# databricks/spark-deep-learning

Hardware: AMD Instinct MI355X
Metric: images/sec (higher is better)
Workload: dtype bf16; 1 GPU; model=resnet50, global_batch=512, image=224, parallelism=dp1

## Files before the change

### sparkdl/models/resnet.py

```python

import torch
import torch.nn as nn

from sparkdl.ops import BatchNormAct2d, Conv1x1, batch_norm_relu_maxpool


class Bottleneck(nn.Module):
    expansion = 4

    def __init__(self, cin, width, stride=1):
        super().__init__()
        cout = width * self.expansion
        self.conv1 = Conv1x1(cin, width)
        self.bn1 = BatchNormAct2d(width, relu=True)
        self.conv2 = nn.Conv2d(width, width, 3, stride=stride, padding=1,
                               bias=False)
        self.bn2 = BatchNormAct2d(width, relu=True)
        self.conv3 = Conv1x1(width, cout)
        self.bn3 = BatchNormAct2d(cout, relu=True)
        if stride != 1 or cin != cout:
            self.down_conv = Conv1x1(cin, cout, stride=stride)
            self.down_bn = BatchNormAct2d(cout, relu=False)
        else:
            self.down_conv = None

    def forward(self, x):
        x, skip = x if isinstance(x, tuple) else (x, x)
        if self.down_conv is not None:
            idn = self.down_bn(self.down_conv(skip))
        else:
            idn = skip
        out = self.bn1(self.conv1(x))
        out = self.bn2(self.conv2(out))
        return self.bn3(self.conv3(out), residual=idn, fork=True)


class ResNet50(nn.Module):
    LAYERS = (3, 4, 6, 3)

    def __init__(self, num_classes=1000):
        super().__init__()
        self.stem_conv = nn.Conv2d(3, 64, 7, stride=2, padding=3,
                                   bias=False)
        self.stem_bn = BatchNormAct2d(64, relu=True)
        self.stem_pool = nn.MaxPool2d(3, stride=2, padding=1)
        cin = 64
        stages = []
        for i, blocks in enumerate(self.LAYERS):
            width = 64 * (2 ** i)
            stride = 1 if i == 0 else 2
            layer = []
            for b in range(blocks):
                layer.append(Bottleneck(cin, width, stride if b == 0 else 1))
                cin = width * Bottleneck.expansion
            stages.append(nn.Sequential(*layer))
        self.stages = nn.Sequential(*stages)
        self.pool = nn.AdaptiveAvgPool2d(1)
        self.fc = nn.Linear(2048, num_classes)

        for m in self.modules():
            if isinstance(m, nn.Conv2d):
                nn.init.kaiming_normal_(m.weight, mode="fan_out",
                                        nonlinearity="relu")
        for m in self.modules():
            if isinstance(m, Bottleneck):
                nn.init.zeros_(m.bn3.weight)

    def forward(self, x):
        bn = self.stem_bn
        x = batch_norm_relu_maxpool(
            self.stem_conv(x), bn.weight, bn.bias, bn.running_mean,
            bn.running_var, momentum=bn.momentum, eps=bn.eps,
            training=bn.training)
        x, _ = self.stages(x)
        x = self.pool(x).flatten(1)
        return self.fc(x)
```

### sparkdl/ops/__init__.py

```python

_EXT = None
_EXT_ERR = None


def ext():
    global _EXT, _EXT_ERR
    if _EXT is None and _EXT_ERR is None:
        try:
            from sparkdl import _C
            _EXT = _C
        except ImportError as e:
            _EXT_ERR = e
    if _EXT is None:
        raise RuntimeError(
            "sparkdl._C HIP extension is not built. Run "
            "`python setup.py build_ext --inplace` (gfx950). "
            "Original error: %s" % _EXT_ERR)
    return _EXT


def has_ext():
    try:
        ext()
        return True
    except RuntimeError:
        return False


from sparkdl.ops.functional import (
    layer_norm, bias_gelu, batch_norm_act, batch_norm_relu_maxpool,
    layer_norm_ref, bias_gelu_ref,
    flash_attention, flash_attention_packed, masked_attention_ref,
    seqlens_from_mask, dropout_add_layer_norm, dropout_keep_mask,
)
from sparkdl.ops.modules import (
    LayerNorm, Linear, LinearGelu, Conv1x1, BatchNormAct2d,
    DropoutAddLayerNorm, convert_bf16_training,
)
from sparkdl.ops.optim import FusedAdamW, FusedSGD
```

### sparkdl/ops/csrc/batchnorm.hip

```cpp

#include "common.hip.h"
#include "kernels.h"

namespace {

constexpr int kBlock = 256;
constexpr int kVec = 8;
constexpr int kUnroll = 2;
constexpr int kFoldFloats = kBlock * 2 * kVec;
constexpr int kFinCh = 4;

__device__ __forceinline__ float bn_affine(short x, float scale,
                                           float shift) {
  return bf2f(x) * scale + shift;
}
__device__ __forceinline__ float bn_xhat(short x, float mean, float rstd) {
  return (bf2f(x) - mean) * rstd;
}
__device__ __forceinline__ float bn_dx(float d, float xh, float k1,
                                       float k2, float k3) {
  return k1 * (d - k2 - xh * k3);
}


// ... 675 lines not shown
      const float k2 = j < 4 ? b0[j] : b1[j - 4];
      const float k3 = j < 4 ? g0[j] : g1[j - 4];
      odx[j] = f2bf(bn_dx(d[j], xh, k1, k2, k3));
    }
    *(short8*)(dx + base) = odx;
  }
}

int bn_grid(long long rows, int cols) {
  const int tpr = cols / kVec;
  const int rpb = kBlock / min(tpr, kBlock);
  long long blocks = (rows + rpb - 1) / rpb;
  return (int)min(blocks, 2048LL);
}

}

int bn_reduce_blocks(long long rows, int cols) {
  const int tpr = cols / kVec;
  const int rpb = kBlock / min(tpr, kBlock);
  const long long row_blocks = (rows + rpb - 1) / rpb;
  const long long g = max(256LL, min(512LL, rows / 64));
  return (int)max(1LL, min(row_blocks, g));
}

long long bn_scratch_floats(long long rows, int cols) {
  return (long long)bn_reduce_blocks(rows, cols) * 2 * cols + 3LL * cols;
}

void launch_bn_fwd(const short* x, const short* res, const float* gamma,
                   const float* beta, float* running_mean,
                   float* running_var, float* save_mean, float* save_rstd,
                   float* scratch, short* y, unsigned char* mask,
                   long long rows, int cols, float momentum, float eps,
                   bool training, bool relu, hipStream_t stream) {
  const int grid = bn_grid(rows, cols);
  const int G = bn_reduce_blocks(rows, cols);
  if (training)
    hipLaunchKernelGGL(bn_stats_k<kUnroll>, dim3(G), dim3(kBlock), 0,
                       stream, x, scratch, rows, cols);
  float* scale = scratch + (size_t)G * 2 * cols;
  float* shift = scale + cols;
  hipLaunchKernelGGL(bn_finalize_k, dim3(cols / kFinCh), dim3(kBlock), 0,
                     stream, scratch, G, gamma, beta, running_mean,
                     running_var, save_mean, save_rstd, scale, shift, rows,
                     cols, momentum, eps, (int)training);
  auto ap = relu ? (res ? bn_apply_k<true, true> : bn_apply_k<true, false>)
                 : (res ? bn_apply_k<false, true>
                        : bn_apply_k<false, false>);
  hipLaunchKernelGGL(ap, dim3(grid), dim3(kBlock), 0, stream, x, res,
                     scale, shift, y, mask, rows, cols);
}

void launch_bn_bwd(const short* x, const unsigned char* mask,
                   const short* dy, const float* gamma,
                   const float* save_mean, const float* save_rstd,
                   float* scratch, float* dgamma, float* dbeta, short* dx,
                   short* dres, long long rows, int cols, bool training,
                   bool relu, hipStream_t stream) {
  const int grid = bn_grid(rows, cols);
  const int G = bn_reduce_blocks(rows, cols);
  auto rk = relu ? bn_bwd_reduce_k<true, kUnroll>
                 : bn_bwd_reduce_k<false, kUnroll>;
  hipLaunchKernelGGL(rk, dim3(G), dim3(kBlock), 0, stream, x, mask, dy,
                     save_mean, save_rstd, scratch, rows, cols);
  float* c1 = scratch + (size_t)G * 2 * cols;
  float* c2 = c1 + cols;
  float* c3 = c2 + cols;
  hipLaunchKernelGGL(bn_bwd_finalize_k, dim3(cols / kFinCh), dim3(kBlock),
                     0, stream, scratch, G, gamma, save_rstd, dgamma, dbeta,
                     c1, c2, c3, rows, cols, (int)training);
  auto ak = relu ? (dres ? bn_bwd_apply_k<true, true>
                         : bn_bwd_apply_k<true, false>)
                 : (dres ? bn_bwd_apply_k<false, true>
                         : bn_bwd_apply_k<false, false>);
  hipLaunchKernelGGL(ak, dim3(grid), dim3(kBlock), 0, stream, x, mask, dy,
                     save_mean, save_rstd, c1, c2, c3, dx, dres, rows,
                     cols);
}

void launch_bn_bwd2(const short* x, const unsigned char* mask,
                    const short* dya, const short* dyb, const float* gamma,
                    const float* save_mean, const float* save_rstd,
                    float* scratch, float* dgamma, float* dbeta, short* dx,
                    short* s, long long rows, int cols, bool training,
                    bool relu, hipStream_t stream) {
  const int grid = bn_grid(rows, cols);
  const int G = bn_reduce_blocks(rows, cols);
  auto rk = relu ? bn_bwd2_reduce_k<true, kUnroll>
                 : bn_bwd2_reduce_k<false, kUnroll>;
  hipLaunchKernelGGL(rk, dim3(G), dim3(kBlock), 0, stream, x, mask, dya,
                     dyb, save_mean, save_rstd, s, scratch, rows, cols);
  float* c1 = scratch + (size_t)G * 2 * cols;
  float* c2 = c1 + cols;
  float* c3 = c2 + cols;
  hipLaunchKernelGGL(bn_bwd_finalize_k, dim3(cols / kFinCh), dim3(kBlock),
                     0, stream, scratch, G, gamma, save_rstd, dgamma, dbeta,
                     c1, c2, c3, rows, cols, (int)training);
  hipLaunchKernelGGL(bn_bwd2_apply_k, dim3(grid), dim3(kBlock), 0, stream,
                     x, s, save_mean, save_rstd, c1, c2, c3, dx, rows,
                     cols);
}

void launch_bn_pool_fwd(const short* x, const float* gamma,
                        const float* beta, float* running_mean,
                        float* running_var, float* save_mean,
// ... 45 lines not shown
```

### sparkdl/ops/csrc/bindings.cpp

```cpp

#include <torch/extension.h>
#include <ATen/hip/impl/HIPStreamMasqueradingAsCUDA.h>
#include <ATen/hip/impl/HIPGuardImplMasqueradingAsCUDA.h>

#include <cmath>
#include <utility>
#include <vector>

#include "kernels.h"

namespace {

using DeviceGuard = c10::hip::HIPGuardMasqueradingAsCUDA;

hipStream_t cur_stream() {
  return c10::hip::getCurrentHIPStreamMasqueradingAsCUDA().stream();
}

#define CHECK_BF16_CUDA(t)                                            \
  TORCH_CHECK((t).is_cuda(), #t " must be on GPU");                   \
  TORCH_CHECK((t).scalar_type() == at::kBFloat16, #t " must be bf16");\
  TORCH_CHECK((t).is_contiguous(), #t " must be contiguous")

#define CHECK_F32_CUDA(t)                                             \
// ... 100 lines not shown
                       dbeta_part.data_ptr<float>(), blocks, rows, cols,
                       cur_stream());
  launch_layernorm_reduce_parts(
      dgamma_part.data_ptr<float>(), dbeta_part.data_ptr<float>(),
      dgamma.data_ptr<float>(), dbeta.data_ptr<float>(), ws_rows, cols,
      cur_stream());
  return {dx, dgamma, dbeta};
}


std::vector<at::Tensor> bn_fwd(const at::Tensor& x,
                               const c10::optional<at::Tensor>& res,
                               const at::Tensor& gamma,
                               const at::Tensor& beta,
                               at::Tensor running_mean,
                               at::Tensor running_var, double momentum,
                               double eps, bool training, bool relu) {
  CHECK_BF16_CUDA(x);
  CHECK_F32_CUDA(gamma);
  CHECK_F32_CUDA(beta);
  DeviceGuard guard(x.device());
  const int cols = (int)x.size(-1);
  const long long rows = x.numel() / cols;
  TORCH_CHECK(cols % 8 == 0 && cols <= 2048,
              "bn_fwd requires cols%8==0 and cols<=2048 (NHWC channels)");
  const short* res_ptr = nullptr;
  if (res.has_value()) {
    CHECK_BF16_CUDA(res.value());
    TORCH_CHECK(res->sizes() == x.sizes());
    res_ptr = bf_ptr(res.value());
  }
  auto f32 = x.options().dtype(at::kFloat);
  auto y = at::empty_like(x);
  auto save_mean = at::empty({cols}, f32);
  auto save_rstd = at::empty({cols}, f32);
  auto scratch = at::empty({bn_scratch_floats(rows, cols)}, f32);
  at::Tensor mask;
  unsigned char* mask_ptr = nullptr;
  if (relu) {
    mask = at::empty({rows * cols / 8}, x.options().dtype(at::kByte));
    mask_ptr = mask.data_ptr<unsigned char>();
  } else {
    mask = at::empty({0}, x.options().dtype(at::kByte));
  }
  launch_bn_fwd(bf_ptr(x), res_ptr, gamma.data_ptr<float>(),
                beta.data_ptr<float>(), running_mean.data_ptr<float>(),
                running_var.data_ptr<float>(), save_mean.data_ptr<float>(),
                save_rstd.data_ptr<float>(), scratch.data_ptr<float>(),
                bf_ptr_mut(y), mask_ptr, rows, cols, (float)momentum,
                (float)eps, training, relu, cur_stream());
  return {y, save_mean, save_rstd, mask};
}

std::vector<at::Tensor> bn_bwd(const at::Tensor& x,
                               const at::Tensor& mask,
                               const at::Tensor& dy,
                               const at::Tensor& gamma,
                               const at::Tensor& save_mean,
                               const at::Tensor& save_rstd, bool training,
                               bool relu, bool needs_dres) {
  CHECK_BF16_CUDA(x);
  CHECK_BF16_CUDA(dy);
  CHECK_F32_CUDA(gamma);
  DeviceGuard guard(x.device());
  const int cols = (int)x.size(-1);
  const long long rows = x.numel() / cols;
  TORCH_CHECK(!relu || mask.numel() == rows * cols / 8,
              "relu backward needs the forward's activation mask");
  auto f32 = x.options().dtype(at::kFloat);
  auto dx = at::empty_like(x);
  auto dgamma = at::empty({cols}, f32);
  auto dbeta = at::empty({cols}, f32);
  auto scratch = at::empty({bn_scratch_floats(rows, cols)}, f32);
  at::Tensor dres;
  short* dres_ptr = nullptr;
  if (needs_dres) {
    dres = at::empty_like(x);
    dres_ptr = bf_ptr_mut(dres);
  }
  launch_bn_bwd(bf_ptr(x),
                relu ? mask.data_ptr<unsigned char>() : nullptr,
                bf_ptr(dy), gamma.data_ptr<float>(),
                save_mean.data_ptr<float>(), save_rstd.data_ptr<float>(),
                scratch.data_ptr<float>(), dgamma.data_ptr<float>(),
                dbeta.data_ptr<float>(), bf_ptr_mut(dx), dres_ptr, rows,
                cols, training, relu, cur_stream());
  if (needs_dres) return {dx, dgamma, dbeta, dres};
  return {dx, dgamma, dbeta};
}

std::vector<at::Tensor> bn_bwd2(const at::Tensor& x,
                                const at::Tensor& mask,
                                const at::Tensor& dy_a,
                                const at::Tensor& dy_b,
                                const at::Tensor& gamma,
                                const at::Tensor& save_mean,
                                const at::Tensor& save_rstd, bool training,
                                bool relu) {
  CHECK_BF16_CUDA(x);
  CHECK_BF16_CUDA(dy_a);
  CHECK_BF16_CUDA(dy_b);
  CHECK_F32_CUDA(gamma);
  TORCH_CHECK(dy_a.sizes() == x.sizes() && dy_b.sizes() == x.sizes(),
              "bn_bwd2: both gradients must have x's shape");
  DeviceGuard guard(x.device());
  const int cols = (int)x.size(-1);
// ... 130 lines not shown
  TORCH_CHECK(cols <= 16384, "bias_gelu_bwd LDS partials support cols<=16384");
  auto dx = at::empty_like(x);
  auto dbias = at::zeros({cols}, x.options().dtype(at::kFloat));
  launch_bias_gelu_bwd(bf_ptr(x), bias.data_ptr<float>(), bf_ptr(dy),
                       bf_ptr_mut(dx), dbias.data_ptr<float>(), rows, cols,
                       cur_stream());
  return {dx, dbias};
}


std::vector<at::Tensor> gemm_bias_act(const at::Tensor& A,
                                      const at::Tensor& W,
                                      const c10::optional<at::Tensor>& bias,
                                      int64_t act, bool save_z) {
  CHECK_BF16_CUDA(A);
  CHECK_BF16_CUDA(W);
  TORCH_CHECK(A.dim() == 2 && W.dim() == 2 && A.size(1) == W.size(1));
  const int M = (int)A.size(0), K = (int)A.size(1), N = (int)W.size(0);
  TORCH_CHECK(gemm_bias_act_supported(M, N, K),
              "gemm_bias_act requires K % 64 == 0");
  const float* bias_ptr = nullptr;
  if (bias.has_value()) {
    CHECK_F32_CUDA(bias.value());
    TORCH_CHECK(bias->numel() == N);
    bias_ptr = bias->data_ptr<float>();
  }
  DeviceGuard guard(A.device());
  auto C = at::empty({M, N}, A.options());
  at::Tensor Z;
  short* z_ptr = nullptr;
  if (save_z && act != 0) {
    Z = at::empty({M, N}, A.options());
    z_ptr = bf_ptr_mut(Z);
  }
  launch_gemm_bias_act(bf_ptr(A), bf_ptr(W), bias_ptr, bf_ptr_mut(C),
                       z_ptr, M, N, K, (int)act, cur_stream());
  if (z_ptr) return {C, Z};
  return {C};
}

at::Tensor gemm_stream(const at::Tensor& A, const at::Tensor& W) {
  CHECK_BF16_CUDA(A);
  CHECK_BF16_CUDA(W);
  TORCH_CHECK(A.dim() == 2 && W.dim() == 2 && A.size(1) == W.size(1));
  const long long M = A.size(0);
  const int K = (int)A.size(1), N = (int)W.size(0);
  TORCH_CHECK(gemm_stream_supported(M, N, K),
              "gemm_stream requires K in {64,128,256} and N % 64 == 0");
  DeviceGuard guard(A.device());
  auto C = at::empty({M, N}, A.options());
  launch_gemm_stream(bf_ptr(A), bf_ptr(W), bf_ptr_mut(C), M, N, K,
                     cur_stream());
  return C;
}


static const long long* seed_ptr(const c10::optional<at::Tensor>& seed) {
  if (!seed.has_value()) return nullptr;
  TORCH_CHECK(seed->is_cuda() && seed->scalar_type() == at::kLong &&
              seed->numel() >= 1);
  return reinterpret_cast<const long long*>(seed->data_ptr<int64_t>());
}

static const int* seqlens_ptr(const c10::optional<at::Tensor>& seqlens,
                              const at::Tensor& like, int64_t rows) {
  if (!seqlens.has_value()) return nullptr;
  TORCH_CHECK(seqlens->is_cuda(), "seqlens must be on GPU");
  TORCH_CHECK(seqlens->device() == like.device(),
              "seqlens must be on the same device as the data");
  TORCH_CHECK(seqlens->scalar_type() == at::kInt,
              "seqlens must be int32");
  TORCH_CHECK(seqlens->is_contiguous(), "seqlens must be contiguous");
  TORCH_CHECK(seqlens->numel() == rows, "seqlens must hold ", rows,
              " entries, got ", seqlens->numel());
  return seqlens->data_ptr<int>();
}

std::vector<at::Tensor> attn_fwd(const at::Tensor& Q, const at::Tensor& K,
                                 const at::Tensor& V, double dropout_p,
                                 const c10::optional<at::Tensor>& seed,
                                 const c10::optional<at::Tensor>& seqlens) {
  CHECK_BF16_CUDA(Q);
  CHECK_BF16_CUDA(K);
  CHECK_BF16_CUDA(V);
  TORCH_CHECK(Q.dim() == 3 && Q.size(2) == 64 && Q.sizes() == K.sizes() &&
                  Q.sizes() == V.sizes(),
              "attn_fwd expects [BH, S, 64] bf16 q/k/v");
  const int BH = (int)Q.size(0), S = (int)Q.size(1);
  TORCH_CHECK(S % 64 == 0, "attn_fwd requires S % 64 == 0");
  TORCH_CHECK(dropout_p == 0.0 || seed.has_value(),
              "dropout needs a seed tensor");
  const int* lens = seqlens_ptr(seqlens, Q, BH);
  DeviceGuard guard(Q.device());
  auto O = at::empty_like(Q);
  auto LSE = at::empty({BH, S}, Q.options().dtype(at::kFloat));
  auto VT = at::empty({BH, 64, S}, Q.options());
  launch_attn_pretranspose(bf_ptr(V), bf_ptr_mut(VT), BH, S, 1, 64,
                           cur_stream());
  launch_attn_fwd(bf_ptr(Q), bf_ptr(K), bf_ptr(VT), bf_ptr_mut(O),
                  LSE.data_ptr<float>(), seed_ptr(seed), BH, S, 1, 64,
                  64, (float)dropout_p, lens, cur_stream());
  return {O, LSE};
}

std::vector<at::Tensor> attn_fwd_packed(
    const at::Tensor& qkv, double dropout_p,
// ... 222 lines not shown
        mean.data_ptr<float>(), rstd.data_ptr<float>(), bf_ptr_mut(d_res),
        bf_ptr_mut(d_sub), dgamma_part.data_ptr<float>(),
        dbeta_part.data_ptr<float>(), blocks, rows, cols, (float)p,
        seed_ptr(seed), cur_stream());
  } else {
    launch_layernorm_bwd(bf_ptr(h), bf_ptr(dy), gamma.data_ptr<float>(),
                         mean.data_ptr<float>(), rstd.data_ptr<float>(),
                         bf_ptr_mut(d_res), dgamma_part.data_ptr<float>(),
                         dbeta_part.data_ptr<float>(), blocks, rows, cols,
                         cur_stream());
  }
  launch_layernorm_reduce_parts(
      dgamma_part.data_ptr<float>(), dbeta_part.data_ptr<float>(),
      dgamma.data_ptr<float>(), dbeta.data_ptr<float>(), ws_rows, cols,
      cur_stream());
  return {d_sub, d_res, dgamma, dbeta};
}


at::Tensor gbt_histogram(const at::Tensor& B, const at::Tensor& g,
                         const at::Tensor& h, const at::Tensor& row_list,
                         const at::Tensor& bmap, int64_t n_nodes) {
  TORCH_CHECK(B.is_cuda() && B.scalar_type() == at::kByte &&
              B.is_contiguous());
  CHECK_F32_CUDA(g);
  CHECK_F32_CUDA(h);
  TORCH_CHECK(row_list.is_cuda() && row_list.scalar_type() == at::kInt);
  TORCH_CHECK(bmap.is_cuda() && bmap.scalar_type() == at::kInt &&
              bmap.size(-1) == 4);
  DeviceGuard guard(B.device());
  const int F = (int)B.size(1);
  TORCH_CHECK(F % 8 == 0, "feature dim must be padded to a multiple of 8");
  auto hist = at::zeros({n_nodes, F, 256, 2},
                        B.options().dtype(at::kFloat));
  launch_gbt_histogram(
      B.data_ptr<unsigned char>(), g.data_ptr<float>(),
      h.data_ptr<float>(), row_list.data_ptr<int>(),
      reinterpret_cast<const int4*>(bmap.data_ptr<int>()),
      (int)(bmap.numel() / 4), F, hist.data_ptr<float>(), cur_stream());
  return hist;
}

}

PYBIND11_MODULE(TORCH_EXTENSION_NAME, m) {
  m.doc() = "sparkdl MI355X-native kernels (gfx950)";
  m.def("fused_adamw_", &fused_adamw_, "Fused multi-tensor AdamW step");
  m.def("fused_sgd_", &fused_sgd_, "Fused multi-tensor SGD step");
  m.def("zero_grads_", &zero_grads_, "Zero all grads in a chunk table");
  m.def("gemm_bias_act", &gemm_bias_act, "MFMA GEMM + bias(+GELU) (N6)");
  m.def("transpose_bf16", &transpose_bf16, "bf16 2D transpose (dgrad W^T)");
  m.def("gemm_stream", &gemm_stream,
        "Streaming tall-skinny GEMM (1x1 convs)");
  m.def("wgrad_splitk", &wgrad_splitk,
        "Split-M wgrad GEMM (tr_b16 fragment path)");
  m.def("attn_fwd", &attn_fwd, "Flash attention fwd (D=64, bf16)",
        py::arg("q"), py::arg("k"), py::arg("v"), py::arg("dropout_p"),
        py::arg("seed"), py::arg("seqlens") = py::none());
  m.def("attn_bwd", &attn_bwd, "Flash attention bwd (dQ/dK/dV)",
        py::arg("q"), py::arg("k"), py::arg("v"), py::arg("dO"),
        py::arg("lse"), py::arg("drow"), py::arg("dropout_p"),
        py::arg("seed"), py::arg("seqlens") = py::none());
  m.def("attn_fwd_packed", &attn_fwd_packed,
        "Flash attention fwd over the packed qkv buffer", py::arg("qkv"),
        py::arg("dropout_p"), py::arg("seed"),
        py::arg("seqlens") = py::none());
  m.def("attn_bwd_packed", &attn_bwd_packed,
        "Flash attention bwd -> packed dqkv", py::arg("qkv"),
        py::arg("dO"), py::arg("lse"), py::arg("drow"),
        py::arg("dropout_p"), py::arg("seed"),
        py::arg("seqlens") = py::none());
  m.def("gbt_histogram", &gbt_histogram, "GBT g/h histogram (N7)");
  m.def("bn_fwd", &bn_fwd, "Fused BatchNorm(+add)(+ReLU) fwd (bf16 NHWC)");
  m.def("bn_bwd", &bn_bwd, "Fused BatchNorm(+add)(+ReLU) bwd (bf16 NHWC)");
  m.def("bn_bwd2", &bn_bwd2,
        "Fused BatchNorm(+add)(+ReLU) bwd over the sum of two gradients");
  m.def("bn_pool_fwd", &bn_pool_fwd,
        "Fused BatchNorm+ReLU+MaxPool(3,2,1) fwd (bf16 NHWC)");
  m.def("bn_pool_bwd", &bn_pool_bwd,
        "Fused BatchNorm+ReLU+MaxPool(3,2,1) bwd (bf16 NHWC)");
  m.def("layernorm_fwd", &layernorm_fwd, "LayerNorm forward (bf16)");
  m.def("layernorm_bwd", &layernorm_bwd, "LayerNorm backward (bf16)");
  m.def("dropout_add_ln_fwd", &dropout_add_ln_fwd,
        "ln(res + dropout(sub)) forward (bf16) -> y, h, mean, rstd",
        py::arg("sub"), py::arg("res"), py::arg("gamma"), py::arg("beta"),
        py::arg("eps"), py::arg("p"), py::arg("seed") = py::none());
  m.def("dropout_add_ln_bwd", &dropout_add_ln_bwd,
        "ln(res + dropout(sub)) backward -> d_sub, d_res, dgamma, dbeta",
        py::arg("h"), py::arg("dy"), py::arg("gamma"), py::arg("mean"),
        py::arg("rstd"), py::arg("p"), py::arg("seed") = py::none());
  m.def("bias_gelu_fwd", &bias_gelu_fwd, "Fused bias+GELU forward (bf16)");
  m.def("bias_gelu_bwd", &bias_gelu_bwd, "Fused bias+GELU backward (bf16)");
  m.attr("_chunk_elems") = kOptChunk;
}
```

### sparkdl/ops/csrc/kernels.h

```cpp
#pragma once

#include <hip/hip_runtime.h>
#include <cstdint>

struct TensorChunk {
  float* p;
  const float* g;
  float* m;
  float* v;
  long long n;
  short* pl;
};

constexpr int kOptChunk = 16384;

void launch_fused_adamw(const TensorChunk* chunks, const int2* bmap,
                        int nblocks, float lr, float beta1, float beta2,
                        float eps, float weight_decay,
                        long long* step_counter, float* coeffs,
                        hipStream_t stream);

void launch_fused_sgd(const TensorChunk* chunks, const int2* bmap,
                      int nblocks, float lr, float momentum,
                      float weight_decay, bool nesterov, bool first_step,
                      hipStream_t stream);

void launch_layernorm_fwd(const short* x, const float* gamma,
                          const float* beta, short* y, float* save_mean,
                          float* save_rstd, int rows, int cols, float eps,
                          hipStream_t stream);

void launch_layernorm_bwd(const short* x, const short* dy,
                          const float* gamma, const float* save_mean,
                          const float* save_rstd, short* dx,
                          float* dgamma_part, float* dbeta_part,
                          int part_rows, int rows, int cols,
                          hipStream_t stream);

int layernorm_bwd_part_rows(int rows);

void launch_layernorm_reduce_parts(const float* dgamma_part,
                                   const float* dbeta_part, float* dgamma,
                                   float* dbeta, int part_rows, int cols,
                                   hipStream_t stream);

void launch_dropout_add_ln_fwd(const short* sub, const short* res,
                               const float* gamma, const float* beta,
                               short* y, short* h, float* save_mean,
                               float* save_rstd, int rows, int cols,
                               float eps, float p, const long long* seed,
                               hipStream_t stream);

void launch_dropout_add_ln_bwd(const short* h, const short* dy,
                               const float* gamma, const float* save_mean,
                               const float* save_rstd, short* d_res,
                               short* d_sub, float* dgamma_part,
                               float* dbeta_part, int part_rows, int rows,
                               int cols, float p, const long long* seed,
                               hipStream_t stream);

void launch_bias_gelu_fwd(const short* x, const float* bias, short* y,
                          long long rows, int cols, hipStream_t stream);

void launch_bias_gelu_bwd(const short* x, const float* bias,
                          const short* dy, short* dx, float* dbias,
                          long long rows, int cols, hipStream_t stream);

int bn_reduce_blocks(long long rows, int cols);
long long bn_scratch_floats(long long rows, int cols);

void launch_bn_fwd(const short* x, const short* res, const float* gamma,
                   const float* beta, float* running_mean,
                   float* running_var, float* save_mean, float* save_rstd,
                   float* scratch, short* y, unsigned char* mask,
                   long long rows, int cols, float momentum, float eps,
                   bool training, bool relu, hipStream_t stream);

void launch_bn_bwd(const short* x, const unsigned char* mask,
                   const short* dy, const float* gamma,
                   const float* save_mean, const float* save_rstd,
                   float* scratch, float* dgamma, float* dbeta, short* dx,
                   short* dres, long long rows, int cols, bool training,
                   bool relu, hipStream_t stream);

void launch_bn_bwd2(const short* x, const unsigned char* mask,
                    const short* dya, const short* dyb, const float* gamma,
                    const float* save_mean, const float* save_rstd,
                    float* scratch, float* dgamma, float* dbeta, short* dx,
                    short* s, long long rows, int cols, bool training,
                    bool relu, hipStream_t stream);

void launch_bn_pool_fwd(const short* x, const float* gamma,
                        const float* beta, float* running_mean,
                        float* running_var, float* save_mean,
                        float* save_rstd, float* scratch, short* pooled,
                        unsigned char* code, int n, int h, int w, int cols,
                        float momentum, float eps, bool training,
                        hipStream_t stream);

void launch_bn_pool_bwd(const short* x, const unsigned char* code,
                        const short* dyp, const float* gamma,
                        const float* save_mean, const float* save_rstd,
                        float* scratch, float* dgamma, float* dbeta,
                        short* dx, int n, int h, int w, int cols,
                        bool training, hipStream_t stream);

void launch_gemm_bias_act(const short* A, const short* W,
                          const float* bias, short* C, short* Z, int M,
                          int N, int K, int act, hipStream_t stream);
bool gemm_bias_act_supported(int M, int N, int K);

void launch_gemm_stream(const short* A, const short* W, short* C,
                        long long M, int N, int K, hipStream_t stream);
bool gemm_stream_supported(long long M, int N, int K);

void launch_wgrad_splitk(const short* dZ, const short* X, float* dW,
                         long long M, int N, int K, hipStream_t stream);
bool wgrad_splitk_supported(long long M, int N, int K);

void launch_transpose_bf16(const short* X, short* Y, int R, int C,
                           hipStream_t stream);

void launch_attn_pretranspose(const short* X, short* T, int BH, int S,
                              int H, int rs, hipStream_t stream);
void launch_attn_fwd(const short* Q, const short* K, const short* VT,
                     short* O, float* LSE, const long long* seed, int BH,
                     int S, int H, int rs, int ors, float dropout_p,
                     const int* seqlens, hipStream_t stream);
void launch_attn_bwd(const short* Q, const short* K, const short* V,
                     const short* dO, const short* QT, const short* DOT,
                     const short* KT, const float* LSE, const float* Drow,
                     short* dQ, short* dK, short* dV,
                     const long long* seed, int BH, int S, int H, int rs,
                     int ors, int grs, float dropout_p,
                     const int* seqlens, hipStream_t stream);

void launch_gbt_histogram(const unsigned char* B, const float* g,
                          const float* h, const int* row_list,
                          const int4* bmap, int nblocks, int F,
                          float* hist, hipStream_t stream);

void launch_zero_grads(const TensorChunk* chunks, const int2* bmap,
                       int nblocks, hipStream_t stream);
```

### sparkdl/ops/functional.py

```python

import os

import torch

import sparkdl.ops as _ops



def layer_norm_ref(x, gamma, beta, eps=1e-5):
    xf = x.float()
    out = torch.nn.functional.layer_norm(
        xf, (x.shape[-1],), gamma.float(), beta.float(), eps)
    return out.to(x.dtype)


def bias_gelu_ref(x, bias):
    return torch.nn.functional.gelu(
        x.float() + bias.float(), approximate="none").to(x.dtype)


def masked_attention_ref(q, k, v, seq_lens, dropout_p=0.0):
    S, d = q.shape[-2], q.shape[-1]
    qf, kf, vf = q.float(), k.float(), v.float()
    lens = torch.as_tensor(seq_lens, device=q.device).clamp(0, S)
# ... 34 lines not shown


class _LayerNormFn(torch.autograd.Function):
    @staticmethod
    def forward(ctx, x, gamma, beta, eps):
        C = _ops.ext()
        x = x.contiguous()
        y, mean, rstd = C.layernorm_fwd(x, gamma, beta, eps)
        ctx.save_for_backward(x, gamma, mean, rstd)
        return y

    @staticmethod
    def backward(ctx, dy):
        C = _ops.ext()
        x, gamma, mean, rstd = ctx.saved_tensors
        dx, dgamma, dbeta = C.layernorm_bwd(
            x, dy.contiguous(), gamma, mean, rstd)
        return dx, dgamma, dbeta, None


class _BiasGeluFn(torch.autograd.Function):
    @staticmethod
    def forward(ctx, x, bias):
        C = _ops.ext()
        x = x.contiguous()
        ctx.save_for_backward(x, bias)
        return C.bias_gelu_fwd(x, bias)

    @staticmethod
    def backward(ctx, dy):
        C = _ops.ext()
        x, bias = ctx.saved_tensors
        dx, dbias = C.bias_gelu_bwd(x, bias, dy.contiguous())
        return dx, dbias


def _to_nhwc(t):
    return t.permute(0, 2, 3, 1).contiguous(memory_format=torch.contiguous_format)


def _from_nhwc(t):
    return t.permute(0, 3, 1, 2)


def _alias(t):
    return torch.empty(0, dtype=t.dtype, device=t.device).set_(
        t.untyped_storage(), t.storage_offset(), t.size(), t.stride())


class _BNReLUFn(torch.autograd.Function):

    @staticmethod
    def forward(ctx, x, residual, gamma, beta, running_mean, running_var,
                momentum, eps, training, relu, fork=False):
        C = _ops.ext()
        xp = _to_nhwc(x)
        rp = _to_nhwc(residual) if residual is not None else None
        y, mean, rstd, mask = C.bn_fwd(
            xp, rp, gamma, beta, running_mean, running_var, momentum,
            eps, training, relu)
        ctx.save_for_backward(xp, mask, gamma, mean, rstd)
        ctx.bn_flags = (training, relu, residual is not None)
        out = _from_nhwc(y)
        if not fork:
            return out
        ctx.set_materialize_grads(False)
        return _alias(out), _alias(out)

    @staticmethod
    def backward(ctx, dy, dy2=None):
        C = _ops.ext()
        xp, mask, gamma, mean, rstd = ctx.saved_tensors
        training, relu, has_res = ctx.bn_flags
        needs_dres = has_res and ctx.needs_input_grad[1]
        if dy is None:
            dy, dy2 = dy2, None
        if dy is None:
            return (None,) * 11
        if dy2 is not None:
            outs = C.bn_bwd2(xp, mask, _to_nhwc(dy), _to_nhwc(dy2), gamma,
                             mean, rstd, training, relu)
        else:
            outs = C.bn_bwd(xp, mask, _to_nhwc(dy), gamma, mean, rstd,
                            training, relu, needs_dres)
        dx = _from_nhwc(outs[0])
        dres = _from_nhwc(outs[3]) if needs_dres else None
        return (dx, dres, outs[1], outs[2], None, None, None, None, None,
                None, None)


def batch_norm_act(x, gamma, beta, running_mean, running_var,
                   momentum=0.1, eps=1e-5, training=True, relu=False,
                   residual=None, fork=False):
    C = x.shape[1]
    if (x.is_cuda and x.dtype == torch.bfloat16
            and C <= 2048 and C % 8 == 0):
        if fork and os.environ.get("SPARKDL_FUSED_RESGRAD", "1") != "0":
            return _BNReLUFn.apply(x, residual, gamma, beta, running_mean,
                                   running_var, momentum, eps, training,
                                   relu, True)
        y = _BNReLUFn.apply(x, residual, gamma, beta, running_mean,
                            running_var, momentum, eps, training, relu,
                            False)
        return (y, y) if fork else y
    y = torch.nn.functional.batch_norm(
        x.float(), running_mean, running_var, gamma, beta,
        training, momentum, eps).to(x.dtype)
    if residual is not None:
        y = y + residual
    y = torch.relu(y) if relu else y
    return (y, y) if fork else y


class _BNReLUPoolFn(torch.autograd.Function):

    @staticmethod
    def forward(ctx, x, gamma, beta, running_mean, running_var, momentum,
                eps, training):
        C = _ops.ext()
        xp = _to_nhwc(x)
        pooled, mean, rstd, code = C.bn_pool_fwd(
            xp, gamma, beta, running_mean, running_var, momentum, eps,
            training)
        ctx.save_for_backward(xp, code, gamma, mean, rstd)
        ctx.bn_training = training
        return _from_nhwc(pooled)

    @staticmethod
    def backward(ctx, dy):
        C = _ops.ext()
        xp, code, gamma, mean, rstd = ctx.saved_tensors
        dx, dgamma, dbeta = C.bn_pool_bwd(
            xp, code, _to_nhwc(dy), gamma, mean, rstd, ctx.bn_training)
        return _from_nhwc(dx), dgamma, dbeta, None, None, None, None, None


def batch_norm_relu_maxpool(x, gamma, beta, running_mean, running_var,
                            momentum=0.1, eps=1e-5, training=True):
    C = x.shape[1]
    if (x.is_cuda and x.dtype == torch.bfloat16 and x.dim() == 4
            and C <= 2048 and C % 8 == 0
            and 0 < x.numel() // C < 2 ** 31
            and os.environ.get("SPARKDL_FUSED_STEM", "1") != "0"):
        return _BNReLUPoolFn.apply(x, gamma, beta, running_mean,
                                   running_var, momentum, eps, training)
    y = batch_norm_act(x, gamma, beta, running_mean, running_var,
                       momentum=momentum, eps=eps, training=training,
                       relu=True)
    return torch.nn.functional.max_pool2d(y, 3, stride=2, padding=1)


def layer_norm(x, gamma, beta, eps=1e-5):
    if x.is_cuda and x.dtype == torch.bfloat16:
        return _LayerNormFn.apply(x, gamma, beta, eps)
    return torch.nn.functional.layer_norm(
        x, (x.shape[-1],), gamma.to(x.dtype), beta.to(x.dtype), eps)

# ... 228 lines not shown


def _wgrad(dz, x2d):
    if (os.environ.get("SPARKDL_FUSED_WGRAD", "0") == "1"
            and dz.shape[1] % 256 == 0 and x2d.shape[1] % 128 == 0
            and dz.shape[0] % 64 == 0):
        C = _ops.ext()
        return C.wgrad_splitk(dz, x2d).to(dz.dtype)
    return dz.t() @ x2d


def _wgrad_splitk(dy, x2d, chunk_rows=32768):
    M = dy.shape[0]
    if M <= 2 * chunk_rows:
        return dy.t() @ x2d
    S = 0
    for s in range((M + chunk_rows - 1) // chunk_rows, 257):
        if M % s == 0:
            S = s
            break
    if S == 0:
        return dy.t() @ x2d
    cr = M // S
    dyb = dy.view(S, cr, -1).transpose(1, 2)
    xb = x2d.view(S, cr, -1)
    return torch.bmm(dyb, xb).sum(0, dtype=torch.float32).to(dy.dtype)


class _Conv1x1Fn(torch.autograd.Function):

    @staticmethod
    def forward(ctx, x2d, weight):
        ctx.save_for_backward(x2d, weight)
        return _conv_gemm(x2d, weight)

    @staticmethod
    def backward(ctx, dy):
        C = _ops.ext()
        x2d, weight = ctx.saved_tensors
        dy = dy.contiguous()
        wt = C.transpose_bf16(weight)
        dx = _conv_gemm(dy, wt)
        dw = _wgrad_splitk(dy, x2d)
        return dx, dw


def conv1x1_gemm(x_nhwc, weight):
    shape = x_nhwc.shape
    x2d = x_nhwc.reshape(-1, shape[-1]).contiguous()
    y = _Conv1x1Fn.apply(x2d, weight.contiguous())
    return y.reshape(*shape[:-1], weight.shape[0])


class _LinearFusedFn(torch.autograd.Function):

    @staticmethod
    def forward(ctx, x2d, weight, bias):
        C = _ops.ext()
        y = C.gemm_bias_act(x2d, weight, bias, 0, False)[0]
        ctx.save_for_backward(x2d, weight)
        ctx.has_bias = bias is not None
        return y

    @staticmethod
    def backward(ctx, dy):
        C = _ops.ext()
        x2d, weight = ctx.saved_tensors
        dy = dy.contiguous()
        if (weight.shape[0] % 64 == 0
                and os.environ.get("SPARKDL_FUSED_DGRAD", "1") != "0"):
            wt = C.transpose_bf16(weight)
            dx = C.gemm_bias_act(dy, wt, None, 0, False)[0]
        else:
            dx = dy @ weight
        dw = _wgrad(dy, x2d)
        dbias = dy.sum(0, dtype=torch.float32) if ctx.has_bias else None
        return dx, dw, dbias


def linear_fused(x, weight, bias):
    shape = x.shape
    x2d = x.reshape(-1, shape[-1]).contiguous()
    y = _LinearFusedFn.apply(x2d, weight.contiguous(), bias)
    return y.reshape(*shape[:-1], weight.shape[0])
```

Measured before the change: 9987 images/s.

## Fuse BatchNorm statistics reduction into 1x1 conv forward GEMM epilogue

Adds a 1x1-conv MFMA kernel that writes its output and, in the same pass, accumulates per-channel sum and sum-of-squares into a partial-sum slab. BatchNorm forward then runs only the finalize and apply kernels on that slab, which removes a separate stats kernel that re-read the activation. It is routed for selected ResNet-50 bottleneck channel pairs in training. Backward now uses aten convolution_backward instead of the custom dgrad/wgrad path, which may be slower, and stats are computed from bf16-rounded outputs.

```diff
diff --git a/sparkdl/models/resnet.py b/sparkdl/models/resnet.py
--- a/sparkdl/models/resnet.py
+++ b/sparkdl/models/resnet.py
@@ -2,7 +2,8 @@
 import torch
 import torch.nn as nn
 
-from sparkdl.ops import BatchNormAct2d, Conv1x1, batch_norm_relu_maxpool
+from sparkdl.ops import (BatchNormAct2d, Conv1x1, batch_norm_relu_maxpool,
+                         conv1x1_bn_act)
 
 
 class Bottleneck(nn.Module):
@@ -27,12 +28,13 @@
     def forward(self, x):
         x, skip = x if isinstance(x, tuple) else (x, x)
         if self.down_conv is not None:
-            idn = self.down_bn(self.down_conv(skip))
+            idn = conv1x1_bn_act(skip, self.down_conv, self.down_bn)
         else:
             idn = skip
-        out = self.bn1(self.conv1(x))
+        out = conv1x1_bn_act(x, self.conv1, self.bn1)
         out = self.bn2(self.conv2(out))
-        return self.bn3(self.conv3(out), residual=idn, fork=True)
+        return conv1x1_bn_act(out, self.conv3, self.bn3, residual=idn,
+                              fork=True)
 
 
 class ResNet50(nn.Module):
diff --git a/sparkdl/ops/__init__.py b/sparkdl/ops/__init__.py
--- a/sparkdl/ops/__init__.py
+++ b/sparkdl/ops/__init__.py
@@ -32,6 +32,7 @@
     layer_norm_ref, bias_gelu_ref,
     flash_attention, flash_attention_packed, masked_attention_ref,
     seqlens_from_mask, dropout_add_layer_norm, dropout_keep_mask,
+    conv1x1_bn_act,
 )
 from sparkdl.ops.modules import (
     LayerNorm, Linear, LinearGelu, Conv1x1, BatchNormAct2d,
diff --git a/sparkdl/ops/csrc/batchnorm.hip b/sparkdl/ops/csrc/batchnorm.hip
--- a/sparkdl/ops/csrc/batchnorm.hip
+++ b/sparkdl/ops/csrc/batchnorm.hip
@@ -751,6 +751,27 @@
                      scale, shift, y, mask, rows, cols);
 }
 
+void launch_bn_fwd_slab(const short* x, const short* res,
+                        const float* slab, int G, const float* gamma,
+                        const float* beta, float* running_mean,
+                        float* running_var, float* save_mean,
+                        float* save_rstd, float* coef, short* y,
+                        unsigned char* mask, long long rows, int cols,
+                        float momentum, float eps, bool relu,
+                        hipStream_t stream) {
+  float* scale = coef;
+  float* shift = coef + cols;
+  hipLaunchKernelGGL(bn_finalize_k, dim3(cols / kFinCh), dim3(kBlock), 0,
+                     stream, slab, G, gamma, beta, running_mean,
+                     running_var, save_mean, save_rstd, scale, shift, rows,
+                     cols, momentum, eps, 1);
+  auto ap = relu ? (res ? bn_apply_k<true, true> : bn_apply_k<true, false>)
+                 : (res ? bn_apply_k<false, true>
+                        : bn_apply_k<false, false>);
+  hipLaunchKernelGGL(ap, dim3(bn_grid(rows, cols)), dim3(kBlock), 0, stream,
+                     x, res, scale, shift, y, mask, rows, cols);
+}
+
 void launch_bn_bwd(const short* x, const unsigned char* mask,
                    const short* dy, const float* gamma,
                    const float* save_mean, const float* save_rstd,
diff --git a/sparkdl/ops/csrc/bindings.cpp b/sparkdl/ops/csrc/bindings.cpp
--- a/sparkdl/ops/csrc/bindings.cpp
+++ b/sparkdl/ops/csrc/bindings.cpp
@@ -176,6 +176,61 @@
   return {y, save_mean, save_rstd, mask};
 }
 
+std::vector<at::Tensor> bn_fwd_slab(const at::Tensor& x,
+                                    const c10::optional<at::Tensor>& res,
+                                    const at::Tensor& slab,
+                                    const at::Tensor& gamma,
+                                    const at::Tensor& beta,
+                                    at::Tensor running_mean,
+                                    at::Tensor running_var, double momentum,
+                                    double eps, bool relu) {
+  CHECK_BF16_CUDA(x);
+  CHECK_F32_CUDA(slab);
+  CHECK_F32_CUDA(gamma);
+  CHECK_F32_CUDA(beta);
+  CHECK_F32_CUDA(running_mean);
+  CHECK_F32_CUDA(running_var);
+  DeviceGuard guard(x.device());
+  const int cols = (int)x.size(-1);
+  const long long rows = x.numel() / cols;
+  TORCH_CHECK(cols % 8 == 0 && cols <= 2048,
+              "bn_fwd_slab requires cols%8==0 and cols<=2048");
+  TORCH_CHECK(slab.dim() == 2 && slab.size(0) >= 1 &&
+                  slab.size(1) == 2 * (int64_t)cols &&
+                  slab.device() == x.device(),
+              "bn_fwd_slab: slab must be [G, 2*cols] on x's device");
+  TORCH_CHECK(gamma.numel() == cols && beta.numel() == cols &&
+              running_mean.numel() == cols && running_var.numel() == cols);
+  const short* res_ptr = nullptr;
+  if (res.has_value()) {
+    CHECK_BF16_CUDA(res.value());
+    TORCH_CHECK(res->sizes() == x.sizes());
+    res_ptr = bf_ptr(res.value());
+  }
+  auto f32 = x.options().dtype(at::kFloat);
+  auto y = at::empty_like(x);
+  auto save_mean = at::empty({cols}, f32);
+  auto save_rstd = at::empty({cols}, f32);
+  auto coef = at::empty({2 * (int64_t)cols}, f32);
+  at::Tensor mask;
+  unsigned char* mask_ptr = nullptr;
+  if (relu) {
+    mask = at::empty({rows * cols / 8}, x.options().dtype(at::kByte));
+    mask_ptr = mask.data_ptr<unsigned char>();
+  } else {
+    mask = at::empty({0}, x.options().dtype(at::kByte));
+  }
+  launch_bn_fwd_slab(bf_ptr(x), res_ptr, slab.data_ptr<float>(),
+                     (int)slab.size(0), gamma.data_ptr<float>(),
+                     beta.data_ptr<float>(), running_mean.data_ptr<float>(),
+                     running_var.data_ptr<float>(),
+                     save_mean.data_ptr<float>(),
+                     save_rstd.data_ptr<float>(), coef.data_ptr<float>(),
+                     bf_ptr_mut(y), mask_ptr, rows, cols, (float)momentum,
+                     (float)eps, relu, cur_stream());
+  return {y, save_mean, save_rstd, mask};
+}
+
 std::vector<at::Tensor> bn_bwd(const at::Tensor& x,
                                const at::Tensor& mask,
                                const at::Tensor& dy,
@@ -412,6 +467,47 @@
   launch_gemm_stream(bf_ptr(A), bf_ptr(W), bf_ptr_mut(C), M, N, K,
                      cur_stream());
   return C;
+}
+
+std::vector<at::Tensor> conv1x1_stats(
+    const at::Tensor& A, const at::Tensor& W, int64_t max_workers,
+    const c10::optional<at::Tensor>& slab_out) {
+  CHECK_BF16_CUDA(A);
+  CHECK_BF16_CUDA(W);
+  TORCH_CHECK(A.dim() == 2 && W.dim() == 2 && A.size(1) == W.size(1));
+  TORCH_CHECK(W.device() == A.device());
+  const long long M = A.size(0);
+  const int K = (int)A.size(1), N = (int)W.size(0);
+  TORCH_CHECK(conv1x1_stats_supported(M, N, K),
+              "conv1x1_stats requires K in {64,128,256}, N % 64 == 0 and "
+              "M >= 1");
+  TORCH_CHECK(max_workers >= 0 && max_workers < (1 << 20));
+  DeviceGuard guard(A.device());
+  int nch, G;
+  conv1x1_stats_plan(M, N, K, (int)max_workers, &nch, &G);
+  auto C = at::empty({M, N}, A.options());
+  at::Tensor slab;
+  if (slab_out.has_value()) {
+    slab = slab_out.value();
+    CHECK_F32_CUDA(slab);
+    TORCH_CHECK(slab.device() == A.device() && slab.dim() == 2 &&
+                    slab.size(0) == G && slab.size(1) == 2 * (int64_t)N,
+                "conv1x1_stats: slab must be [", G, ", ", 2 * N, "]");
+  } else {
+    slab = at::empty({G, 2 * (int64_t)N}, A.options().dtype(at::kFloat));
+  }
+  launch_conv1x1_stats(bf_ptr(A), bf_ptr(W), bf_ptr_mut(C),
+                       slab.data_ptr<float>(), M, N, K, (int)max_workers,
+                       cur_stream());
+  return {C, slab};
+}
+
+std::vector<int64_t> conv1x1_stats_plan_py(int64_t M, int64_t N, int64_t K,
+                                           int64_t max_workers) {
+  TORCH_CHECK(conv1x1_stats_supported(M, (int)N, (int)K));
+  int nch, G;
+  conv1x1_stats_plan(M, (int)N, (int)K, (int)max_workers, &nch, &G);
+  return {nch, G};
 }
 
 
@@ -740,6 +836,16 @@
   m.def("transpose_bf16", &transpose_bf16, "bf16 2D transpose (dgrad W^T)");
   m.def("gemm_stream", &gemm_stream,
         "Streaming tall-skinny GEMM (1x1 convs)");
+  m.def("conv1x1_stats", &conv1x1_stats,
+        "Read-once 1x1 conv forward + BatchNorm partial sums -> C, slab",
+        py::arg("a"), py::arg("w"), py::arg("max_workers") = 0,
+        py::arg("slab") = py::none());
+  m.def("conv1x1_stats_plan", &conv1x1_stats_plan_py,
+        "(chunks per N-block, slab rows G) of a conv1x1_stats launch",
+        py::arg("m"), py::arg("n"), py::arg("k"),
+        py::arg("max_workers") = 0);
+  m.def("bn_fwd_slab", &bn_fwd_slab,
+        "Fused BatchNorm(+add)(+ReLU) fwd over pre-summed statistics");
   m.def("wgrad_splitk", &wgrad_splitk,
         "Split-M wgrad GEMM (tr_b16 fragment path)");
   m.def("attn_fwd", &attn_fwd, "Flash attention fwd (D=64, bf16)",
diff --git a/sparkdl/ops/csrc/conv1x1_stats.hip b/sparkdl/ops/csrc/conv1x1_stats.hip
--- /dev/null
+++ b/sparkdl/ops/csrc/conv1x1_stats.hip
@@ -0,0 +1,223 @@
+
+#include "mfma_tile.hip.h"
+#include "kernels.h"
+
+namespace {
+
+constexpr int CTHREADS = 1024;
+constexpr int CWAVES = CTHREADS / 64;
+constexpr int CCH = 64;
+constexpr int kMaxPanel = 128 * 1024;
+constexpr int kCUs = 256;
+
+__device__ __forceinline__ void wave_lds_sync() {
+  __builtin_amdgcn_fence(__ATOMIC_RELEASE, "wavefront");
+  __builtin_amdgcn_wave_barrier();
+  __builtin_amdgcn_fence(__ATOMIC_ACQUIRE, "wavefront");
+}
+
+template <int K, int R, int NCH>
+__global__ __launch_bounds__(CTHREADS) void conv1x1_stats_k(
+    const short* __restrict__ A, const short* __restrict__ W,
+    short* __restrict__ C, float* __restrict__ slab, long long M, int N,
+    int G) {
+  constexpr int NB = NCH * CCH;
+  constexpr int RI = R / 16;
+  constexpr int NTK = K / 32;
+  constexpr int row_shift = K == 64 ? 7 : (K == 128 ? 8 : 9);
+  static_assert(NB * K * 2 <= kMaxPanel, "W panel exceeds its LDS share");
+  static_assert(CWAVES * 2 * NB * 4 <= NB * K * 2, "fold tile fits panel");
+  static_assert(2 * NB <= CTHREADS, "one thread per slab-row entry");
+  __shared__ __attribute__((aligned(16))) short lW[NB * K];
+  __shared__ __attribute__((aligned(16))) short lC[CWAVES * 16 * CCH];
+
+  const int nnb = N / NB;
+  int g, nbk;
+  if (G % 8 == 0) {
+    nbk = (blockIdx.x / 8) % nnb;
+    g = (blockIdx.x / (8 * nnb)) * 8 + blockIdx.x % 8;
+  } else {
+    nbk = blockIdx.x % nnb;
+    g = blockIdx.x / nnb;
+  }
+
+  const int tid = threadIdx.x;
+  const int lane = tid & 63;
+  const int wave = __builtin_amdgcn_readfirstlane(tid >> 6);
+  const FragLane fl(lane);
+
+  for (int e0 = tid * 8; e0 < NB * K; e0 += CTHREADS * 8) {
+    const int e = tile_swz(e0 * 2, row_shift) / 2;
+    const int row = e / K, kk = e % K;
+    global_load_lds16(W + ((long long)nbk * NB + row) * K + kk,
+                      lW + (e0 - lane * 8));
+  }
+  __builtin_amdgcn_s_waitcnt(0);
+  __syncthreads();
+
+  float s[NCH], ss[NCH];
+#pragma unroll
+  for (int ch = 0; ch < NCH; ++ch) s[ch] = ss[ch] = 0.f;
+
+  const long long nblk = (M + R - 1) / R;
+  const long long Q = (long long)G * CWAVES;
+  const long long q = (long long)g * CWAVES + wave;
+  const long long b0 = q * nblk / Q, b1 = (q + 1) * nblk / Q;
+  short* myC = lC + wave * (16 * CCH);
+
+  for (long long blk = b0; blk < b1; ++blk) {
+    const long long m0 = blk * R;
+    bf16x8 a[RI][NTK];
+#pragma unroll
+    for (int i = 0; i < RI; ++i) {
+      long long row = m0 + i * 16 + fl.frag_row;
+      if (row >= M) row = M - 1;
+#pragma unroll
+      for (int ks = 0; ks < NTK; ++ks)
+        a[i][ks] = *(const bf16x8*)(A + row * K + ks * 32 + fl.frag_k);
+    }
+
+#pragma unroll 1
+    for (int ch = 0; ch < NCH; ++ch) {
+      const short* lWc = lW + ch * (CCH * K);
+      f32x4 acc[RI][4];
+#pragma unroll
+      for (int i = 0; i < RI; ++i)
+#pragma unroll
+        for (int j = 0; j < 4; ++j) acc[i][j] = {0.f, 0.f, 0.f, 0.f};
+
+#pragma unroll
+      for (int ks = 0; ks < NTK; ++ks) {
+        __builtin_amdgcn_s_setprio(1);
+#pragma unroll
+        for (int j = 0; j < 4; ++j) {
+          const bf16x8 b = *(const bf16x8*)(
+              (const char*)lWc +
+              tile_swz(((j * 16 + fl.frag_row) * K + ks * 32 + fl.frag_k) * 2,
+                       row_shift));
+#pragma unroll
+          for (int i = 0; i < RI; ++i)
+            acc[i][j] = mfma_bf16(a[i][ks], b, acc[i][j]);
+        }
+        __builtin_amdgcn_s_setprio(0);
+      }
+
+#pragma unroll
+      for (int i = 0; i < RI; ++i) {
+        wave_lds_sync();
+#pragma unroll
+        for (int j = 0; j < 4; ++j)
+#pragma unroll
+          for (int rr = 0; rr < 4; ++rr)
+            myC[(fl.c_sub_row + rr) * CCH + j * 16 + fl.c_col] =
+                f2bf(acc[i][j][rr]);
+        wave_lds_sync();
+        const long long gr0 = m0 + i * 16;
+#pragma unroll
+        for (int t = 0; t < 2; ++t) {
+          const int r = t * 8 + lane / 8;
+          const int c = (lane % 8) * 8;
+          const long long grow = gr0 + r;
+          if (grow < M) {
+            const bf16x8 v = *(const bf16x8*)&myC[r * CCH + c];
+            *(bf16x8*)&C[grow * N + (long long)nbk * NB + ch * CCH + c] = v;
+          }
+        }
+        const long long left = M - gr0;
+        const int nvalid = left >= 16 ? 16 : (left > 0 ? (int)left : 0);
+        float t1 = 0.f, t2 = 0.f;
+#pragma unroll
+        for (int r = 0; r < 16; ++r) {
+          if (r < nvalid) {
+            const float v = bf2f(myC[r * CCH + lane]);
+            t1 += v;
+            t2 += v * v;
+          }
+        }
+#pragma unroll
+        for (int c2 = 0; c2 < NCH; ++c2) {
+          s[c2] += c2 == ch ? t1 : 0.f;
+          ss[c2] += c2 == ch ? t2 : 0.f;
+        }
+      }
+    }
+  }
+
+  __syncthreads();
+  float* red = (float*)lW;
+#pragma unroll
+  for (int ch = 0; ch < NCH; ++ch) {
+    red[(wave * 2 + 0) * NB + ch * CCH + lane] = s[ch];
+    red[(wave * 2 + 1) * NB + ch * CCH + lane] = ss[ch];
+  }
+  __syncthreads();
+  if (tid < 2 * NB) {
+    const int half = tid / NB, c = tid % NB;
+    float t = 0.f;
+#pragma unroll
+    for (int w = 0; w < CWAVES; ++w) t += red[(w * 2 + half) * NB + c];
+    slab[(size_t)g * 2 * N + (size_t)half * N + (size_t)nbk * NB + c] = t;
+  }
+}
+
+constexpr int rows_per_block(int K, int nch) {
+  return K == 256 || (K == 128 && nch >= 4) ? 16 : 32;
+}
+
+template <int K, int NCH>
+void launch_one(const short* A, const short* W, short* C, float* slab,
+                long long M, int N, int G, hipStream_t stream) {
+  const int nnb = N / (NCH * CCH);
+  hipLaunchKernelGGL((conv1x1_stats_k<K, rows_per_block(K, NCH), NCH>),
+                     dim3(G * nnb), dim3(CTHREADS), 0, stream, A, W, C,
+                     slab, M, N, G);
+}
+
+template <int K>
+void launch_k(int nch, const short* A, const short* W, short* C,
+              float* slab, long long M, int N, int G, hipStream_t stream) {
+  if constexpr (K * 8 * CCH * 2 <= kMaxPanel) {
+    if (nch == 8)
+      return launch_one<K, 8>(A, W, C, slab, M, N, G, stream);
+  }
+  if (nch == 4) return launch_one<K, 4>(A, W, C, slab, M, N, G, stream);
+  if (nch == 2) return launch_one<K, 2>(A, W, C, slab, M, N, G, stream);
+  launch_one<K, 1>(A, W, C, slab, M, N, G, stream);
+}
+
+}
+
+bool conv1x1_stats_supported(long long M, int N, int K) {
+  return (K == 64 || K == 128 || K == 256) && N >= CCH && N % CCH == 0 &&
+         M >= 1;
+}
+
+void conv1x1_stats_plan(long long M, int N, int K, int max_workers,
+                        int* nch, int* G) {
+  int c = 8;
+  while (c > 1 && (N % (c * CCH) != 0 || c * CCH * K * 2 > kMaxPanel))
+    c /= 2;
+  const int nnb = N / (c * CCH);
+  const int R = rows_per_block(K, c);
+  long long g = kCUs / nnb / 8 * 8;
+  if (g < 8) g = 8;
+  const long long by_rows = M / ((long long)CWAVES * R);
+  if (g > by_rows) g = by_rows;
+  if (g < 1) g = 1;
+  if (max_workers > 0 && g > max_workers) g = max_workers;
+  *nch = c;
+  *G = (int)g;
+}
+
+void launch_conv1x1_stats(const short* A, const short* W, short* C,
+                          float* slab, long long M, int N, int K,
+                          int max_workers, hipStream_t stream) {
+  int nch, G;
+  conv1x1_stats_plan(M, N, K, max_workers, &nch, &G);
+  if (K == 64)
+    launch_k<64>(nch, A, W, C, slab, M, N, G, stream);
+  else if (K == 128)
+    launch_k<128>(nch, A, W, C, slab, M, N, G, stream);
+  else
+    launch_k<256>(nch, A, W, C, slab, M, N, G, stream);
+}
diff --git a/sparkdl/ops/csrc/kernels.h b/sparkdl/ops/csrc/kernels.h
--- a/sparkdl/ops/csrc/kernels.h
+++ b/sparkdl/ops/csrc/kernels.h
@@ -76,6 +76,15 @@
                    long long rows, int cols, float momentum, float eps,
                    bool training, bool relu, hipStream_t stream);
 
+void launch_bn_fwd_slab(const short* x, const short* res,
+                        const float* slab, int G, const float* gamma,
+                        const float* beta, float* running_mean,
+                        float* running_var, float* save_mean,
+                        float* save_rstd, float* coef, short* y,
+                        unsigned char* mask, long long rows, int cols,
+                        float momentum, float eps, bool relu,
+                        hipStream_t stream);
+
 void launch_bn_bwd(const short* x, const unsigned char* mask,
                    const short* dy, const float* gamma,
                    const float* save_mean, const float* save_rstd,
@@ -114,6 +123,13 @@
                         long long M, int N, int K, hipStream_t stream);
 bool gemm_stream_supported(long long M, int N, int K);
 
+bool conv1x1_stats_supported(long long M, int N, int K);
+void conv1x1_stats_plan(long long M, int N, int K, int max_workers,
+                        int* nch, int* G);
+void launch_conv1x1_stats(const short* A, const short* W, short* C,
+                          float* slab, long long M, int N, int K,
+                          int max_workers, hipStream_t stream);
+
 void launch_wgrad_splitk(const short* dZ, const short* X, float* dW,
                          long long M, int N, int K, hipStream_t stream);
 bool wgrad_splitk_supported(long long M, int N, int K);
diff --git a/sparkdl/ops/functional.py b/sparkdl/ops/functional.py
--- a/sparkdl/ops/functional.py
+++ b/sparkdl/ops/functional.py
@@ -110,13 +110,18 @@
 
     @staticmethod
     def forward(ctx, x, residual, gamma, beta, running_mean, running_var,
-                momentum, eps, training, relu, fork=False):
+                momentum, eps, training, relu, fork=False, slab=None):
         C = _ops.ext()
         xp = _to_nhwc(x)
         rp = _to_nhwc(residual) if residual is not None else None
-        y, mean, rstd, mask = C.bn_fwd(
-            xp, rp, gamma, beta, running_mean, running_var, momentum,
-            eps, training, relu)
+        if slab is not None and training:
+            y, mean, rstd, mask = C.bn_fwd_slab(
+                xp, rp, slab, gamma, beta, running_mean, running_var,
+                momentum, eps, relu)
+        else:
+            y, mean, rstd, mask = C.bn_fwd(
+                xp, rp, gamma, beta, running_mean, running_var, momentum,
+                eps, training, relu)
         ctx.save_for_backward(xp, mask, gamma, mean, rstd)
         ctx.bn_flags = (training, relu, residual is not None)
         out = _from_nhwc(y)
@@ -134,7 +139,7 @@
         if dy is None:
             dy, dy2 = dy2, None
         if dy is None:
-            return (None,) * 11
+            return (None,) * 12
         if dy2 is not None:
             outs = C.bn_bwd2(xp, mask, _to_nhwc(dy), _to_nhwc(dy2), gamma,
                              mean, rstd, training, relu)
@@ -144,23 +149,24 @@
         dx = _from_nhwc(outs[0])
         dres = _from_nhwc(outs[3]) if needs_dres else None
         return (dx, dres, outs[1], outs[2], None, None, None, None, None,
-                None, None)
+                None, None, None)
 
 
 def batch_norm_act(x, gamma, beta, running_mean, running_var,
                    momentum=0.1, eps=1e-5, training=True, relu=False,
-                   residual=None, fork=False):
+                   residual=None, fork=False, slab=None):
     C = x.shape[1]
     if (x.is_cuda and x.dtype == torch.bfloat16
             and C <= 2048 and C % 8 == 0):
         if fork and os.environ.get("SPARKDL_FUSED_RESGRAD", "1") != "0":
             return _BNReLUFn.apply(x, residual, gamma, beta, running_mean,
                                    running_var, momentum, eps, training,
-                                   relu, True)
+                                   relu, True, slab)
         y = _BNReLUFn.apply(x, residual, gamma, beta, running_mean,
                             running_var, momentum, eps, training, relu,
-                            False)
+                            False, slab)
         return (y, y) if fork else y
+    assert slab is None, "a statistics slab needs the kernel path"
     y = torch.nn.functional.batch_norm(
         x.float(), running_mean, running_var, gamma, beta,
         training, momentum, eps).to(x.dtype)
@@ -495,6 +501,68 @@
     return y.reshape(*shape[:-1], weight.shape[0])
 
 
+
+CONV1X1_STATS_SITES = frozenset({
+    (64, 64), (64, 256), (256, 64), (256, 128), (128, 512), (256, 1024),
+})
+
+
+def conv1x1_stats_supported(cin, cout):
+    return cin in (64, 128, 256) and cout >= 64 and cout % 64 == 0
+
+
+def conv1x1_stats_route(cin, cout, stride=1, mode=None):
+    if mode is None:
+        mode = os.environ.get("SPARKDL_CONV1X1_STATS", "1")
+    if mode == "0" or stride != 1 or not conv1x1_stats_supported(cin, cout):
+        return False
+    if os.environ.get("SPARKDL_CONV1X1", "0") == "all":
+        return False
+    return mode == "all" or (cin, cout) in CONV1X1_STATS_SITES
+
+
+class _Conv1x1StatsFn(torch.autograd.Function):
+
+    @staticmethod
+    def forward(ctx, x, weight):
+        C = _ops.ext()
+        n, cin, h, w = x.shape
+        x2d = x.permute(0, 2, 3, 1).reshape(n * h * w, cin)
+        y2d, slab = C.conv1x1_stats(x2d, weight, 0)
+        ctx.save_for_backward(x, weight)
+        ctx.mark_non_differentiable(slab)
+        ctx.set_materialize_grads(False)
+        y = y2d.view(n, h, w, weight.shape[0]).permute(0, 3, 1, 2)
+        return y, slab
+
+    @staticmethod
+    def backward(ctx, dy, _dslab):
+        if dy is None:
+            return None, None
+        x, weight = ctx.saved_tensors
+        w4 = weight.view(weight.shape[0], weight.shape[1], 1, 1)
+        dx, dw, _ = torch.ops.aten.convolution_backward(
+            dy, x, w4, None, [1, 1], [0, 0], [1, 1], False, [0, 0], 1,
+            [ctx.needs_input_grad[0], ctx.needs_input_grad[1], False])
+        if dw is not None:
+            dw = dw.view_as(weight)
+        return dx, dw
+
+
+def conv1x1_bn_act(x, conv, bn, residual=None, fork=False):
+    if (bn.training and x.is_cuda and x.dtype == torch.bfloat16
+            and x.dim() == 4
+            and x.is_contiguous(memory_format=torch.channels_last)
+            and bn.num_features == conv.cout
+            and conv1x1_stats_route(conv.cin, conv.cout, conv.stride)):
+        y, slab = _Conv1x1StatsFn.apply(x, conv.weight.to(x.dtype))
+        return batch_norm_act(
+            y, bn.weight, bn.bias, bn.running_mean, bn.running_var,
+            momentum=bn.momentum, eps=bn.eps, training=True, relu=bn.relu,
+            residual=residual, fork=fork, slab=slab)
+    return bn(conv(x), residual=residual, fork=fork)
+
+
 class _LinearFusedFn(torch.autograd.Function):
 
     @staticmethod
```

Result: faster. 10220 images/s, median of 6 (+2.3%).
